# nhcha6/embodied-object-detection

Hardware: AMD Instinct MI355X
Metric: frames/sec (640x640, implicit_memory); frames/sec/GPU = value / n_gpus (higher is better)
Workload: dtype f32

## Files before the change

embodied_object_detection_amd/build.py:

```python
from __future__ import annotations

import os
import subprocess
import sys

HERE = os.path.dirname(os.path.abspath(__file__))
CSRC = os.path.join(HERE, "csrc")
LIB = os.path.join(HERE, "libeod_hip.so")
SOURCES = ["conv_igemm.hip", "conv_fp32.hip", "conv_pointwise.hip", "conv_bf16x3.hip", "conv_f16.hip", "elementwise.hip", "roi_align.hip", "select.hip", "heads.hip", "memory.hip", "semmap.hip", "place.hip", "regions.hip", "inventory.hip", "memory_read.hip", "memory_backward.hip", "conv_wgrad.hip", "train_losses.hip", "describe.hip", "relations.hip"]
ARCH = "gfx950"


def _stale() -> bool:
    if not os.path.exists(LIB):
        return True
    t = os.path.getmtime(LIB)
    deps = [os.path.join(CSRC, f) for f in os.listdir(CSRC)] + [os.path.join(HERE, "..", "include", h) for h in ("eod_hip.h", "eod_place.h", "eod_regions.h", "eod_inventory.h", "eod_describe.h", "eod_relations.h")]
    return any(os.path.getmtime(d) > t for d in deps if os.path.exists(d))


def _usage_file(src: str) -> str:
    return os.path.join(HERE, "build", src.replace(".hip", ".usage.txt"))


def resource_usage() -> dict:
    import re
    out = {}
    for src in SOURCES:
        f = _usage_file(src)
        if not os.path.exists(f):
            continue
        cur = None
        for line in open(f):
            m = re.search(r"Function Name: (\S+)", line)
            if m:
                cur = out.setdefault(m.group(1), {})
                continue
            for key, pat in (("vgprs", r"\bVGPRs: (\d+)"), ("scratch", r"ScratchSize \[bytes/lane\]: (\d+)"),
                             ("occupancy", r"Occupancy \[waves/SIMD\]: (\d+)"), ("lds", r"LDS Size \[bytes/block\]: (\d+)")):
                m = re.search(pat, line)
                if m and cur is not None:
                    cur[key] = int(m.group(1))
    return out


def scratch_offenders(usage: dict = None) -> list:
    usage = resource_usage() if usage is None else usage
    return sorted(k for k, v in usage.items() if v.get("scratch", 0) > 0)


def build(force: bool = False, verbose: bool = True) -> str:
    if not force and not _stale():
        return LIB
    hipcc = os.environ.get("HIPCC", "/opt/rocm/bin/hipcc")
    objs = []
    procs = []
    os.makedirs(os.path.join(HERE, "build"), exist_ok=True)
    for src in SOURCES:
        obj = os.path.join(HERE, "build", src.replace(".hip", ".o"))
        cmd = [hipcc, f"--offload-arch={ARCH}", "-O3", "-fPIC", "-std=c++17", "-Wall", "-Wno-unused-function",
               "-ffp-contract=on", "-Rpass-analysis=kernel-resource-usage", "-c", os.path.join(CSRC, src), "-o", obj]
        if verbose:
            print(" ".join(cmd), flush=True)
        procs.append((src, subprocess.Popen(cmd, stderr=open(_usage_file(src), "w"))))
        objs.append(obj)
    failed = [s for s, p in procs if p.wait() != 0]
    for src in SOURCES:
        skip = 0
        held = []
        for line in open(_usage_file(src)):
            if line.startswith("In file included from"):
                held.append(line)
                continue
            trace, held = held, []
            if "kernel-resource-usage" in line:
                skip = 2 if "Function Name" in line else 0
                continue
            sys.stderr.writelines(trace)
            if skip and (line.lstrip()[:1].isdigit() or line.strip().startswith("|")):
                skip -= 1
                continue
            skip = 0
            if line.strip():
                sys.stderr.write(line)
    if failed:
        raise RuntimeError(f"hipcc failed for {failed}")
    bad = scratch_offenders()
    if bad:
        raise RuntimeError("kernels that use scratch memory (register spills / an argument struct copied to private memory): " + ", ".join(bad))
    cmd = [hipcc, f"--offload-arch={ARCH}", "-shared", "-fPIC", "-o", LIB] + objs
    if verbose:
        print(" ".join(cmd), flush=True)
    subprocess.check_call(cmd)
    return LIB


if __name__ == "__main__":
    build(force="--force" in sys.argv)
    print(LIB)
```

embodied_object_detection_amd/csrc/conv_common.h:

```cpp
#pragma once
#include "eod_common.h"
#include "conv_border_order.h"
#include "../../include/eod_hip.h"

namespace eodconv {


struct ConvArgs {
  const float* x;
  const float* w;
  const float* bias;
  const float* res;
  const float* gate;
  float* y;
  float* partial;
  const int* m_count;
  int m_unit;
  int m_segs, seg_rows;
  const float* fuse_w;
  const int* out_units;
  float fuse_b;
  int N, H, W, Cin, OH, OW, Cout, KH, KW, stride, pad, Kpad;
  int M, nchunks, splitk, cps;
  int relu, res_mode, in_relu, out_mode;
  int tiles_m, tiles_n;
  float out_scale;
  int nlv;
  int lv_off[EOD_MAX_LEVELS + 1], lv_h[EOD_MAX_LEVELS], lv_w[EOD_MAX_LEVELS];
  unsigned x_bytes, w_bytes;
  const void* w3;
  unsigned w3_bytes;
  const void* wh;
  unsigned wh_bytes;
  double* gn_partial;
  int gn_groups;
  float* y2;
  int split_n;
  FastDiv div_ow, div_oh, div_cd, div_row;
  int border;
  FastDiv div_bh, div_bw, div_bi;
};

__device__ __forceinline__ int conv_row_limit(const ConvArgs& p, int M) {
  if (p.m_count && p.m_segs <= 1) {
    const int lim = *p.m_count * p.m_unit;
    M = lim < M ? lim : M;
  }
  return M;
}

__device__ __forceinline__ bool conv_row_active(const ConvArgs& p, int m) {
  if (!p.m_count || p.m_segs <= 1) return true;
  const int s = m / p.seg_rows;
  return m - s * p.seg_rows < p.m_count[s] * p.m_unit;
}

__device__ __forceinline__ bool conv_tile_active(const ConvArgs& p, int m0, int bm) {
  if (!p.m_count || p.m_segs <= 1) return true;
  const int last = (m0 + bm - 1 < p.M ? m0 + bm - 1 : p.M - 1);
  const int s0 = m0 / p.seg_rows, s1 = last / p.seg_rows;
  if (m0 - s0 * p.seg_rows < p.m_count[s0] * p.m_unit) return true;
  for (int s = s0 + 1; s <= s1; ++s)
    if (p.m_count[s] > 0) return true;
  return false;
}

__device__ __forceinline__ int border_rois(const ConvArgs& p) {
  const int c = *p.m_count;
  return c < p.N ? c : p.N;
}
__device__ __forceinline__ int border_storage_row(const ConvArgs& p, int m, int rois) {
  const BorderRow b = border_row(m, rois, p.OH, p.OW, p.div_ow, p.div_bh, p.div_bw, p.div_bi);
  return (b.img * p.OH + b.oy) * p.OW + b.ox;
}

template <bool GATE = false>
__device__ __forceinline__ float epilogue_store(const ConvArgs& p, float v, int m, int n) {
  int co = n;
  size_t oidx;
  if (p.out_mode == 1) {
    const int Cd = p.Cout >> 2;
    const int quad = (int)fdiv((unsigned)n, p.div_cd);
    co = n - quad * Cd;
    const int dy = quad >> 1, dx = quad & 1;
    const int t = (int)fdiv((unsigned)m, p.div_ow);
    const int ox = m - t * p.OW;
    const int img = (int)fdiv((unsigned)t, p.div_oh);
    const int oy = t - img * p.OH;
    oidx = ((size_t)(img * 2 * p.OH + 2 * oy + dy) * (2 * p.OW) + (2 * ox + dx)) * Cd + co;
  } else {
    oidx = (size_t)m * p.Cout + n;
  }
  if (p.bias) v += p.bias[co];
  v *= p.out_scale;
  if (p.res_mode == 1) {
    v += p.res[(size_t)m * p.Cout + n];
  } else if (p.res_mode == 2) {
    const int t = (int)fdiv((unsigned)m, p.div_ow);
    const int ox = m - t * p.OW;
    const int img = (int)fdiv((unsigned)t, p.div_oh);
    const int oy = t - img * p.OH;
    const int rh = p.OH >> 1, rw = p.OW >> 1;
    v += p.res[((size_t)(img * rh + (oy >> 1)) * rw + (ox >> 1)) * p.Cout + n];
  }
  if (p.split_n > 0) {
    if (n >= p.split_n) {
      if (p.relu) v = fmaxf(v, 0.0f);
      p.y2[(size_t)m * (p.Cout - p.split_n) + (n - p.split_n)] = v;
    } else {
      p.y[(size_t)m * p.split_n + n] = v;
    }
    return v;
  }
  if (p.relu) v = fmaxf(v, 0.0f);
  if (GATE && p.gate && !(p.gate[oidx] > 0.0f)) v = 0.0f;
  p.y[oidx] = v;
  return v;
}

__device__ __forceinline__ unsigned long long tap_mask(int iy0, int ix0, int hh, int ww, int KH, int KW) {
  unsigned long long mask = 0;
  int tp = 0;
  for (int ky = 0; ky < KH; ++ky) {
    const bool rok = (unsigned)(iy0 + ky) < (unsigned)hh;
    for (int kx = 0; kx < KW; ++kx, ++tp) {
      const bool ok = rok && ((unsigned)(ix0 + kx) < (unsigned)ww);
      mask |= (unsigned long long)ok << tp;
    }
  }
  return mask;
}

template <int TM, int TN, bool GATE = false, bool BORDER = false>
__device__ __forceinline__ void store_wave_tiles(const ConvArgs& p, const f32x16 (&acc)[TM][TN], int m_base, int n_base, int M, int z,
                                                 int lane) {
  const int half = lane >> 5;
  const int rois = BORDER ? border_rois(p) : 0;
#pragma unroll
  for (int i = 0; i < TM; ++i) {
#pragma unroll
    for (int j = 0; j < TN; ++j) {
      const int n = n_base + j * 32 + (lane & 31);
#pragma unroll
      for (int r = 0; r < 16; ++r) {
        const int row = (r & 3) + 8 * (r >> 2) + 4 * half;
        const int m = m_base + i * 32 + row;
        if (m < M && n < p.Cout && conv_row_active(p, m)) {
          const float v = acc[i][j][r];
          if (BORDER) {
            epilogue_store<GATE>(p, v, border_storage_row(p, m, rois), n);
          } else if (p.splitk > 1) {
            p.partial[((size_t)z * p.M + m) * p.Cout + n] = v;
          } else {
            epilogue_store<GATE>(p, v, m, n);
          }
        }
      }
    }
  }
}

void launch_conv_fp32(const ConvArgs& a, int tile, int bk, bool tap4, dim3 grid, hipStream_t s, int lds_reserve = 0, int prefetch2 = 0);
void launch_conv_bf16x3(const ConvArgs& a, int tile, dim3 grid, hipStream_t s);
void launch_conv_wavek(const ConvArgs& a, int nw, dim3 grid, hipStream_t s);
void launch_conv_pointwise(const ConvArgs& a, int np, dim3 grid, hipStream_t s);
void launch_split_weights(const float* w, void* out, int Cout, int Kpad, hipStream_t s);
void launch_conv_f16(const ConvArgs& a, int tile, int bk, dim3 grid, hipStream_t s);
void launch_half_weights(const float* w, void* out, int Cout, int Kpad, hipStream_t s);

}
```

embodied_object_detection_amd/csrc/conv_igemm.hip:

```cpp
#include "conv_common.h"
#include "../../include/eod_hip.h"
#include <atomic>
#include <cstdlib>
#include <cstring>

namespace {

using namespace eodconv;

template <int VEC>
__global__ __launch_bounds__(256) void conv_splitk_reduce_kernel(ConvArgs p) {
  EOD_CHAIN_PRIO();
  const int M = conv_row_limit(p, p.M);
  const unsigned per_row = (unsigned)p.Cout / VEC;
  const unsigned total = (unsigned)M * per_row;
  const size_t slab = (size_t)p.M * p.Cout;
  for (unsigned idx = blockIdx.x * blockDim.x + threadIdx.x; idx < total; idx += gridDim.x * blockDim.x) {
    const unsigned m = fdiv(idx, p.div_row);
    if (!conv_row_active(p, (int)m)) continue;
    const unsigned n = (idx - m * per_row) * VEC;
    const float* src = p.partial + (size_t)m * p.Cout + n;
    if (VEC == 4) {
      f32x4 v = {0.f, 0.f, 0.f, 0.f};
      for (int zb = 0; zb < p.splitk; zb += 4) {
        f32x4 t[4];
#pragma unroll
        for (int j = 0; j < 4; ++j)
          if (zb + j < p.splitk) t[j] = *reinterpret_cast<const f32x4*>(src + (size_t)(zb + j) * slab);
#pragma unroll
        for (int j = 0; j < 4; ++j)
          if (zb + j < p.splitk) v += t[j];
      }
      epilogue_store<true>(p, v.x, (int)m, (int)n);
      epilogue_store<true>(p, v.y, (int)m, (int)n + 1);
      epilogue_store<true>(p, v.z, (int)m, (int)n + 2);
      epilogue_store<true>(p, v.w, (int)m, (int)n + 3);
    } else {
      float v = 0.f;
      for (int z = 0; z < p.splitk; ++z) v += src[z * slab];
      epilogue_store<true>(p, v, (int)m, (int)n);
    }
  }
}

#define EOD_GN_ROWS 32
__global__ __launch_bounds__(256) void conv_splitk_reduce_gn_kernel(ConvArgs p) {
  EOD_CHAIN_PRIO();
  __shared__ double red[4][64][2];
  int level = 0, first_chunk = 0;
  for (;;) {
    const int rows = p.lv_off[level + 1] - p.lv_off[level];
    const int nch = (rows + EOD_GN_ROWS - 1) / EOD_GN_ROWS;
    if ((int)blockIdx.x < first_chunk + nch || level + 1 >= p.nlv) break;
    first_chunk += nch;
    ++level;
  }
  const int r0 = p.lv_off[level] + ((int)blockIdx.x - first_chunk) * EOD_GN_ROWS;
  const int r1 = min(r0 + EOD_GN_ROWS, p.lv_off[level + 1]);
  const int C = p.Cout;
  const int c4 = C >> 2;
  const int nsub = 256 / c4;
  const int col = threadIdx.x % c4, sub = threadIdx.x / c4;
  const int cpg4 = (C / p.gn_groups) >> 2;
  const size_t slab = (size_t)p.M * C;
  double s = 0.0, q = 0.0;
  for (int r = r0 + sub; r < r1; r += nsub) {
    const float* src = p.partial + (size_t)r * C + col * 4;
    f32x4 v = {0.f, 0.f, 0.f, 0.f};
    for (int zb = 0; zb < p.splitk; zb += 4) {
      f32x4 t[4];
#pragma unroll
      for (int j = 0; j < 4; ++j)
        if (zb + j < p.splitk) t[j] = *reinterpret_cast<const f32x4*>(src + (size_t)(zb + j) * slab);
#pragma unroll
      for (int j = 0; j < 4; ++j)
        if (zb + j < p.splitk) v += t[j];
    }
    const double o0 = (double)epilogue_store<true>(p, v.x, r, col * 4 + 0);
    const double o1 = (double)epilogue_store<true>(p, v.y, r, col * 4 + 1);
    const double o2 = (double)epilogue_store<true>(p, v.z, r, col * 4 + 2);
    const double o3 = (double)epilogue_store<true>(p, v.w, r, col * 4 + 3);
    s += o0; q += o0 * o0;
    s += o1; q += o1 * o1;
    s += o2; q += o2 * o2;
    s += o3; q += o3 * o3;
  }
  for (int off = 1; off < cpg4; off <<= 1) {
    s += __shfl_xor(s, off, 64);
    q += __shfl_xor(q, off, 64);
  }
  if ((col % cpg4) == 0) {
    red[sub][col / cpg4][0] = s;
    red[sub][col / cpg4][1] = q;
  }
  __syncthreads();
  if ((int)threadIdx.x < p.gn_groups) {
    double ts = 0.0, tq = 0.0;
    for (int u = 0; u < nsub; ++u) {
      ts += red[u][threadIdx.x][0];
      tq += red[u][threadIdx.x][1];
    }
    p.gn_partial[((size_t)blockIdx.x * p.gn_groups + threadIdx.x) * 2 + 0] = ts;
    p.gn_partial[((size_t)blockIdx.x * p.gn_groups + threadIdx.x) * 2 + 1] = tq;
  }
}

std::atomic<int>& math_mode() {
  static std::atomic<int> v([] {
    const char* e = getenv("EOD_CONV_MATH");
    if (e && strcmp(e, "bf16x3") == 0) return EOD_MATH_BF16X3;
    if (e && strcmp(e, "f16") == 0) return EOD_MATH_F16;
    return EOD_MATH_FP32;
  }());
  return v;
}

struct Plan {
  int tile;
  int bk;
  int glds;
  int bm, bn, tiles_m, tiles_n, splitk, cps, nchunks;
  int wavek;
  int pw_np;
  int border;
};

constexpr int kForcePointwise = 30;

int effective_math(const EodConvDesc* d) { return d->math > 0 ? d->math - 1 : math_mode().load(std::memory_order_relaxed); }

bool pointwise_eligible(const EodConvDesc* d) {
  return effective_math(d) == EOD_MATH_FP32 && d->KH == 1 && d->KW == 1 && d->stride == 1 && d->pad == 0 && d->levels <= 0 && !d->tap4 &&
         d->Cin == d->Kpad && (d->Cin == 64 || d->Cin == 128 || d->Cin == 256) && d->Cout % 64 == 0 && d->out_mode == 0 &&
         (d->res_mode == 0 || d->res_mode == 1) && !d->in_relu && !d->gate && !d->m_count && d->split_n == 0 && !d->gn_partial &&
         d->lds_reserve == 0;
}

constexpr int kForceBorder = 43;
constexpr bool kBorderAuto = true;

bool border_eligible(const EodConvDesc* d) {
  return effective_math(d) == EOD_MATH_FP32 && d->KH == 3 && d->KW == 3 && d->stride == 1 && d->pad == 1 && d->levels <= 0 && !d->tap4 &&
         d->m_count && d->m_segments <= 1 && d->m_unit == d->OH * d->OW && d->OH >= 3 && d->OW >= 3 && d->Cin % 32 == 0 &&
         d->out_mode == 0 && d->res_mode == 0 && !d->in_relu && !d->gate && d->split_n == 0 && !d->gn_partial && d->prefetch2 == 0;
}

Plan make_plan(const EodConvDesc* d, int M) {
  static const int cfg[5][2] = {{128, 128}, {128, 64}, {64, 64}, {256, 128}, {64, 256}};
  Plan pl{};
  int pick = 2;
  const int ft = d->force_tile % 10, fbk = d->force_tile / 10;
  const bool half_ok = !d->tap4 && !d->in_relu;
  const bool f16_forced = (fbk == 8 || fbk == 9) && half_ok;
  if (f16_forced) pick = ft == 4 ? 3 : 2;
  else if (ft >= 1 && ft <= 3) pick = ft - 1;
  else if (ft == 4 && fbk == 5 && half_ok) pick = 3;
  const bool bk64_ok = !d->tap4 && d->Cin % 64 == 0 && d->Kpad % 64 == 0;
  pl.glds = f16_forced ? 3 : ((fbk == 5 && half_ok) ? 2 : 0);
  const int Mp = (d->plan_rows > 0 && d->plan_rows < M) ? d->plan_rows : M;
  const int math = effective_math(d);
  if (d->force_tile == 0 && math == EOD_MATH_F16 && half_ok) {
    pl.glds = 3;
    pick = (long)((Mp + 255) / 256) * ((d->Cout + 127) / 128) >= 256 ? 3 : 2;
  }
  if (d->force_tile == 0 && math == EOD_MATH_BF16X3 && half_ok) {
    pl.glds = 2;
    const long t128 = (long)((Mp + 127) / 128) * ((d->Cout + 127) / 128);
    const long t256 = (long)((Mp + 255) / 256) * ((d->Cout + 127) / 128);
    pick = t256 >= 256 ? 3 : (t128 >= 512 ? 0 : 2);
  }
  if (d->out_mode == 2) {
    pick = 4;
    pl.glds = 0;
  }
  if (d->gate) {
    const bool f16_gated = d->math == EOD_MATH_F16 + 1 && half_ok && d->levels <= 0 && (d->force_tile == 0 || f16_forced);
    pick = 2;
    pl.glds = f16_gated ? 3 : 0;
  }
  if (pl.glds == 3) pl.bk = (fbk == 8 && d->Cin % 64 == 0) ? 64 : 32;
  else pl.bk = (pl.glds == 0 && d->out_mode != 2 && fbk == 2 && bk64_ok) ? 64 : 32;
  const int nchunks = d->Kpad / pl.bk;
  pl.nchunks = nchunks;
  pl.tile = pick + 1;
  pl.bm = cfg[pick][0];
  pl.bn = cfg[pick][1];
  pl.tiles_m = (M + pl.bm - 1) / pl.bm;
  pl.tiles_n = (d->Cout + pl.bn - 1) / pl.bn;
  const long tiles = (long)((Mp + pl.bm - 1) / pl.bm) * pl.tiles_n;
  int splitk = 1;
  if (d->out_mode == 2) {
    splitk = 1;
  } else if (d->force_splitk > 0) {
    splitk = d->force_splitk;
  } else if (pl.glds == 0 && !d->tap4 && nchunks >= 8 &&
             ((d->force_tile == 6 || d->force_tile == 7) ||
              (tiles < 256 && nchunks <= 192 && pl.bk == 32 && d->force_tile == 0 &&
               ((Mp <= 512 && nchunks / (nchunks >= 64 ? 8 : 4) >= 8) || nchunks >= 128)))) {
    pl.wavek = d->force_tile == 6 ? 4 : (d->force_tile == 7 ? 8 : (nchunks >= 64 ? 8 : 4));
    pl.bk = 32;
    pl.nchunks = d->Kpad / 32;
    pl.bm = pl.bn = 32;
    pl.tiles_m = (M + 31) / 32;
    pl.tiles_n = (d->Cout + 31) / 32;
  } else if (tiles < 256 && nchunks >= 8) {
    const int target = (nchunks >= 128 && Mp <= 512) ? 1792 : 512;
    int want = (int)((target + tiles - 1) / tiles);
    int maxs = nchunks / 4;
    splitk = want < maxs ? want : maxs;
    if (splitk < 1) splitk = 1;
  } else if (tiles >= 256 && tiles <= 1024 && d->m_count == nullptr && nchunks >= 18) {
    double best = 1e30;
    for (int sct = 1; sct <= 4; ++sct) {
      if (nchunks / sct < 9) break;
      const double est = (double)((tiles * sct + 255) / 256) / sct + (sct > 1 ? 0.12 : 0.0);
      if (est < best - 1e-9) {
        best = est;
        splitk = sct;
      }
    }
  }
  if (splitk > nchunks) splitk = nchunks;
  pl.cps = (nchunks + splitk - 1) / splitk;
  pl.splitk = (nchunks + pl.cps - 1) / pl.cps;
  const bool pw_forced = d->force_tile == kForcePointwise && d->force_splitk <= 1;
  const bool pw_auto = d->force_tile == 0 && d->force_splitk == 0 && pointwise_eligible(d) && pl.splitk == 1 && !pl.wavek && tiles >= 256 &&
                       !(d->Kpad == 256 && d->Cout < 1024);
  if (pw_forced || pw_auto) {
    const int panels = d->Cout / 64;
    const long row_tiles = (Mp + 63) / 64;
    const long want = tiles >= 256 ? 512 : 1;
    int np = 1;
    for (int cand = 4; cand > 1; cand >>= 1)
      if (panels >= cand && row_tiles * ((panels + cand - 1) / cand) >= want) {
        np = cand;
        break;
      }
    pl.pw_np = np;
    pl.tile = 6;
    pl.glds = 0;
    pl.bk = 32;
    pl.nchunks = d->Kpad / 32;
    pl.bm = 64;
    pl.bn = 64 * np;
    pl.tiles_m = (M + 63) / 64;
    pl.tiles_n = (panels + np - 1) / np;
    pl.splitk = 1;
    pl.cps = pl.nchunks;
    pl.wavek = 0;
  }
  const bool border_forced = d->force_tile == kForceBorder && d->force_splitk <= 1;
  const bool border_auto = kBorderAuto && d->force_tile == 0 && border_eligible(d) && pl.glds == 0 && pl.tile == 3 && pl.bk == 32 &&
                           pl.splitk == 1 && !pl.wavek;
  if (border_forced) {
    pl.splitk = 1;
    pl.cps = pl.nchunks;
  }
  pl.border = (border_forced || border_auto) ? 1 : 0;
  return pl;
}

int total_rows(const EodConvDesc* d) { return d->levels > 0 ? d->level_off[d->levels] : d->N * d->OH * d->OW; }

int check_desc(const EodConvDesc* d) {
  if (!d || !d->x || !d->w || !d->y) return EOD_ERR_NULL;
  if (d->N <= 0 || d->Cin <= 0 || d->Cout <= 0) return EOD_ERR_BAD_DIMS;
  if (d->levels <= 0 && (d->H <= 0 || d->W <= 0 || d->OH <= 0 || d->OW <= 0)) return EOD_ERR_BAD_DIMS;
  if (d->KH <= 0 || d->KW <= 0 || d->stride <= 0 || d->pad < 0) return EOD_ERR_BAD_DIMS;
  if (d->Kpad % 32 != 0 || d->Kpad < d->KH * d->KW * d->Cin) return EOD_ERR_BAD_DIMS;
  if (d->tap4) {
    if (d->Cin != 4) return EOD_ERR_BAD_DIMS;
  } else {
    if (d->Cin % 32 != 0 || d->Kpad != d->KH * d->KW * d->Cin) return EOD_ERR_BAD_DIMS;
  }
  if (d->levels > 0) {
    if (d->levels > EOD_MAX_LEVELS || d->N != 1 || d->stride != 1 || d->KH != d->KW || d->pad != d->KH / 2 || d->tap4 || d->out_mode != 0 ||
        d->res_mode == 2 || d->level_off[0] != 0)
      return EOD_ERR_BAD_DIMS;
    for (int l = 0; l < d->levels; ++l)
      if (d->level_h[l] <= 0 || d->level_w[l] <= 0 || d->level_off[l + 1] - d->level_off[l] != d->level_h[l] * d->level_w[l])
        return EOD_ERR_BAD_DIMS;
  } else {
    if (d->OH != (d->H + 2 * d->pad - d->KH) / d->stride + 1) return EOD_ERR_BAD_DIMS;
    if (d->OW != (d->W + 2 * d->pad - d->KW) / d->stride + 1) return EOD_ERR_BAD_DIMS;
  }
  if (d->levels <= 0 && (long)d->N * d->H * d->W * d->Cin >= (1L << 29)) return EOD_ERR_BAD_DIMS;
  if ((long)d->Cout * d->Kpad >= (1L << 29)) return EOD_ERR_BAD_DIMS;
  if (d->KH * d->KW > 64) return EOD_ERR_BAD_DIMS;
  if ((long)total_rows(d) * (d->Cout > d->Cin ? d->Cout : d->Cin) >= (1L << 31)) return EOD_ERR_BAD_DIMS;
  if (d->out_mode == 1 && (d->Cout % 4 != 0)) return EOD_ERR_BAD_DIMS;
  if (d->out_mode == 2) {
    if (d->Cout != 1024 || d->KH != 1 || d->KW != 1 || d->stride != 1 || d->tap4 || d->levels > 0 || d->res_mode != 0 || d->in_relu ||
        d->force_splitk > 1)
      return EOD_ERR_BAD_DIMS;
    if (!d->fuse_w) return EOD_ERR_NULL;
  }
  if (d->out_mode < 0 || d->out_mode > 2) return EOD_ERR_BAD_DIMS;
  if (d->res_mode != 0 && !d->res) return EOD_ERR_NULL;
  if (d->res_mode == 2 && ((d->OH & 1) || (d->OW & 1))) return EOD_ERR_BAD_DIMS;
  if (d->m_count && d->m_unit <= 0) return EOD_ERR_BAD_DIMS;
  if (d->m_segments > 1) {
    if (!d->m_count || d->levels > 0 || d->out_mode == 2 || d->m_segments > EOD_MAX_BATCH || d->N % d->m_segments != 0)
      return EOD_ERR_BAD_DIMS;
    if (((long)(d->N / d->m_segments) * d->OH * d->OW) % d->m_unit != 0) return EOD_ERR_BAD_DIMS;
  }
  if (d->gate && (d->out_mode != 0 || d->split_n != 0 || d->gn_partial)) return EOD_ERR_BAD_DIMS;
  if (d->gate && d->force_tile != 0 && d->force_tile % 10 != 3 && d->force_tile != 6 && d->force_tile != 7) return EOD_ERR_BAD_DIMS;
  if (d->gate && d->force_tile / 10 == 5) return EOD_ERR_BAD_DIMS;
  if (d->gate && (d->force_tile / 10 == 8 || d->force_tile / 10 == 9) &&
      (d->math != EOD_MATH_F16 + 1 || d->force_tile % 10 != 3 || d->levels > 0 || d->tap4 || d->in_relu))
    return EOD_ERR_BAD_DIMS;
  if (d->math < 0 || d->math > EOD_MATH_F16 + 1) return EOD_ERR_BAD_DIMS;
  if ((d->force_tile / 10 == 8 || d->force_tile / 10 == 9) && d->force_tile % 10 != 3 && d->force_tile % 10 != 4) return EOD_ERR_BAD_DIMS;
  if (d->lds_reserve < 0 || d->lds_reserve > 48 * 1024) return EOD_ERR_BAD_DIMS;
  if (d->force_tile == kForcePointwise && (!pointwise_eligible(d) || d->force_splitk > 1)) return EOD_ERR_BAD_DIMS;
  if (d->force_tile == kForceBorder && (!border_eligible(d) || d->force_splitk > 1)) return EOD_ERR_BAD_DIMS;
  if (d->split_n != 0) {
    if (!d->y2) return EOD_ERR_NULL;
    if (d->split_n < 0 || d->split_n >= d->Cout || d->out_mode != 0 || d->res_mode != 0 || d->levels > 0 || d->gn_partial)
      return EOD_ERR_BAD_DIMS;
  }
  if (d->gn_partial) {
    const int cpg = d->gn_groups > 0 ? d->Cout / d->gn_groups : 0;
    if (d->levels <= 0 || d->m_count || d->out_mode != 0 || d->gn_groups <= 0 || d->gn_groups > 64 || d->Cout % d->gn_groups != 0 ||
        cpg > 64 || (cpg & (cpg - 1)) != 0 || cpg < 4 || d->Cout % 4 != 0 || d->Cout > 1024 || 256 % (d->Cout / 4) != 0 ||
        64 % (cpg / 4) != 0)
      return EOD_ERR_BAD_DIMS;
  }
  if (!eod_aligned16(d->x) || !eod_aligned16(d->w) || !eod_aligned16(d->w_split) || !eod_aligned16(d->w_half)) return EOD_ERR_ALIGN;
  return EOD_OK;
}

}

extern "C" int eod_set_conv_math(int mode) {
  if (mode != EOD_MATH_FP32 && mode != EOD_MATH_BF16X3 && mode != EOD_MATH_F16) return EOD_ERR_BAD_DIMS;
  return math_mode().exchange(mode);
}

extern "C" int eod_get_conv_math(void) { return math_mode().load(); }

extern "C" size_t eod_conv_split_weights_bytes(int Cout, int Kpad) {
  return (Cout > 0 && Kpad > 0 && Kpad % 32 == 0) ? (size_t)Cout * Kpad * 6 : 0;
}

extern "C" int eod_conv_split_weights_bf16x3(const float* w, int Cout, int Kpad, void* out, eod_stream_t stream) {
  if (!w || !out) return EOD_ERR_NULL;
  if (Cout <= 0 || Kpad <= 0 || Kpad % 32 != 0 || (long)Cout * Kpad * 6 >= (1L << 32)) return EOD_ERR_BAD_DIMS;
  if (!eod_aligned16(w) || !eod_aligned16(out)) return EOD_ERR_ALIGN;
  launch_split_weights(w, out, Cout, Kpad, static_cast<hipStream_t>(stream));
  return eod_launch_status();
}

extern "C" size_t eod_conv_half_weights_bytes(int Cout, int Kpad) {
  return (Cout > 0 && Kpad > 0 && Kpad % 32 == 0) ? (size_t)Cout * Kpad * 2 : 0;
}

extern "C" int eod_conv_half_weights(const float* w, int Cout, int Kpad, void* out, eod_stream_t stream) {
  if (!w || !out) return EOD_ERR_NULL;
  if (Cout <= 0 || Kpad <= 0 || Kpad % 32 != 0 || (long)Cout * Kpad >= (1L << 29)) return EOD_ERR_BAD_DIMS;
  if (!eod_aligned16(w) || !eod_aligned16(out)) return EOD_ERR_ALIGN;
  launch_half_weights(w, out, Cout, Kpad, static_cast<hipStream_t>(stream));
  return eod_launch_status();
}

extern "C" int eod_conv2d_gn_fused(const EodConvDesc* d) {
  EodConvDesc t = *d;
  t.gn_partial = nullptr;
  if (check_desc(&t) != EOD_OK) return 0;
  return make_plan(&t, total_rows(&t)).splitk > 1 ? 1 : 0;
}

extern "C" int eod_conv2d_plan(const EodConvDesc* d, EodConvPlan* out) {
  if (!out) return EOD_ERR_NULL;
  const int st = check_desc(d);
  if (st != EOD_OK) return st;
  const Plan pl = make_plan(d, total_rows(d));
  out->tile = pl.tile; out->bm = pl.bm; out->bn = pl.bn; out->bk = pl.bk;
  out->splitk = pl.splitk; out->cps = pl.cps; out->nchunks = pl.nchunks;
  out->wavek = pl.wavek; out->glds = pl.glds;
  out->tiles_m = pl.tiles_m; out->tiles_n = pl.tiles_n;
  out->gn_fused = (d->gn_partial && pl.splitk > 1) ? 1 : 0;
  return EOD_OK;
}

extern "C" size_t eod_conv2d_workspace_bytes(const EodConvDesc* d) {
  if (check_desc(d) != EOD_OK) return 0;
  const int M = total_rows(d);
  const Plan pl = make_plan(d, M);
  if (pl.splitk <= 1) return 0;
  return (size_t)pl.splitk * M * d->Cout * sizeof(float);
}

extern "C" int eod_conv2d(const EodConvDesc* d, eod_stream_t stream) {
  const int st = check_desc(d);
  if (st != EOD_OK) return st;
  hipStream_t s = static_cast<hipStream_t>(stream);
  ConvArgs a{};
  a.x = d->x; a.w = d->w; a.bias = d->bias; a.res = d->res; a.y = d->y;
  a.partial = d->workspace;
  a.m_count = d->m_count; a.m_unit = d->m_unit;
  a.m_segs = d->m_segments > 1 ? d->m_segments : 1;
  a.seg_rows = a.m_segs > 1 ? (d->N / d->m_segments) * d->OH * d->OW : 0;
  a.fuse_w = d->fuse_w; a.out_units = d->out_units; a.fuse_b = d->fuse_b;
  a.N = d->N; a.H = d->H; a.W = d->W; a.Cin = d->Cin; a.OH = d->OH; a.OW = d->OW; a.Cout = d->Cout;
  a.KH = d->KH; a.KW = d->KW; a.stride = d->stride; a.pad = d->pad; a.Kpad = d->Kpad;
  a.M = total_rows(d);
  a.div_ow = eod_make_fastdiv((unsigned)(d->OW > 0 ? d->OW : 1));
  a.div_oh = eod_make_fastdiv((unsigned)(d->OH > 0 ? d->OH : 1));
  a.div_row = eod_make_fastdiv((unsigned)(d->Cout % 4 == 0 ? d->Cout / 4 : d->Cout));
  a.div_cd = eod_make_fastdiv((unsigned)((d->Cout >> 2) > 0 ? (d->Cout >> 2) : 1));
  a.div_bh = eod_make_fastdiv((unsigned)(d->OH > 2 ? d->OH - 2 : 1));
  a.div_bw = eod_make_fastdiv((unsigned)(d->OW > 2 ? d->OW - 2 : 1));
  a.div_bi = eod_make_fastdiv((unsigned)(d->OH > 2 && d->OW > 2 ? (d->OH - 2) * (d->OW - 2) : 1));
  {
    const size_t xe = d->levels > 0 ? (size_t)d->level_off[d->levels] * d->Cin : (size_t)d->N * d->H * d->W * d->Cin;
    a.x_bytes = (unsigned)(xe * sizeof(float));
    a.w_bytes = (unsigned)((size_t)d->Cout * d->Kpad * sizeof(float));
    a.w3 = d->w_split;
    a.w3_bytes = (unsigned)((size_t)d->Cout * d->Kpad * 6);
    a.wh = d->w_half;
    a.wh_bytes = (unsigned)((size_t)d->Cout * d->Kpad * 2);
  }
  a.nlv = d->levels > 0 ? d->levels : 0;
  for (int l = 0; l < a.nlv; ++l) {
    a.lv_off[l] = d->level_off[l];
    a.lv_h[l] = d->level_h[l];
    a.lv_w[l] = d->level_w[l];
  }
  if (a.nlv) a.lv_off[a.nlv] = d->level_off[a.nlv];
  a.relu = d->relu; a.res_mode = d->res_mode; a.in_relu = d->in_relu; a.out_mode = d->out_mode;
  a.gate = d->gate;
  a.out_scale = d->out_scale;
  a.gn_partial = d->gn_partial;
  a.gn_groups = d->gn_groups;
  a.y2 = d->y2;
  a.split_n = d->split_n;
  const Plan pl = make_plan(d, a.M);
  if (d->gn_partial && pl.splitk <= 1) return EOD_ERR_BAD_DIMS;
  a.nchunks = pl.nchunks;
  a.splitk = pl.splitk; a.cps = pl.cps; a.tiles_m = pl.tiles_m; a.tiles_n = pl.tiles_n;
  a.border = pl.border;
  if (pl.splitk > 1) {
    const size_t need = (size_t)pl.splitk * a.M * a.Cout * sizeof(float);
    if (!d->workspace || d->workspace_bytes < need) return EOD_ERR_CAPACITY;
  }
  dim3 grid(pl.tiles_m * pl.tiles_n, pl.splitk);
  if (pl.border) grid.x = (pl.tiles_m + 7) / 8 * 8 * pl.tiles_n;
  if (pl.pw_np) launch_conv_pointwise(a, pl.pw_np, grid, s);
  else if (pl.wavek) launch_conv_wavek(a, pl.wavek, grid, s);
  else if (pl.glds == 3) launch_conv_f16(a, pl.tile, pl.bk, grid, s);
  else if (pl.glds == 2) launch_conv_bf16x3(a, pl.tile, grid, s);
  else launch_conv_fp32(a, pl.tile, pl.bk, d->tap4 != 0, grid, s, d->lds_reserve, d->prefetch2);
  if (pl.splitk > 1) {
    const size_t total = (size_t)a.M * a.Cout;
    const bool vec = a.Cout % 4 == 0;
    int blocks = (int)((total / (vec ? 4 : 1) + 255) / 256);
    if (blocks > 2048) blocks = 2048;
    if (blocks < 1) blocks = 1;
    if (a.gn_partial) {
      int chunks = 0;
      for (int l = 0; l < a.nlv; ++l) chunks += (a.lv_off[l + 1] - a.lv_off[l] + EOD_GN_ROWS - 1) / EOD_GN_ROWS;
      hipLaunchKernelGGL(conv_splitk_reduce_gn_kernel, dim3(chunks), dim3(256), 0, s, a);
    } else if (vec) hipLaunchKernelGGL(conv_splitk_reduce_kernel<4>, dim3(blocks), dim3(256), 0, s, a);
    else hipLaunchKernelGGL(conv_splitk_reduce_kernel<1>, dim3(blocks), dim3(256), 0, s, a);
  }
  return eod_launch_status();
}
```

Before: 325.9.

## Add narrow-Cout 3x3 conv kernel with in-block split-K reduction

Adds a dedicated kernel for 3x3 stride-1 FP32 convolutions with at most 8 output channels. It is chosen automatically whenever the planner would otherwise use split-K. Each block covers 64 rows, and its four waves each take a K partition. Weights are broadcast across lanes with readlane, and the partial sums are reduced in LDS inside the block. This removes the split-K workspace write and the separate reduction kernel that the generic tiled path uses for these heads, but it may lose parallelism when there are few rows.

```diff
diff --git a/embodied_object_detection_amd/build.py b/embodied_object_detection_amd/build.py
--- a/embodied_object_detection_amd/build.py
+++ b/embodied_object_detection_amd/build.py
@@ -7,7 +7,7 @@
 HERE = os.path.dirname(os.path.abspath(__file__))
 CSRC = os.path.join(HERE, "csrc")
 LIB = os.path.join(HERE, "libeod_hip.so")
-SOURCES = ["conv_igemm.hip", "conv_fp32.hip", "conv_pointwise.hip", "conv_bf16x3.hip", "conv_f16.hip", "elementwise.hip", "roi_align.hip", "select.hip", "heads.hip", "memory.hip", "semmap.hip", "place.hip", "regions.hip", "inventory.hip", "memory_read.hip", "memory_backward.hip", "conv_wgrad.hip", "train_losses.hip", "describe.hip", "relations.hip"]
+SOURCES = ["conv_igemm.hip", "conv_fp32.hip", "conv_pointwise.hip", "conv_narrow.hip", "conv_bf16x3.hip", "conv_f16.hip", "elementwise.hip", "roi_align.hip", "select.hip", "heads.hip", "memory.hip", "semmap.hip", "place.hip", "regions.hip", "inventory.hip", "memory_read.hip", "memory_backward.hip", "conv_wgrad.hip", "train_losses.hip", "describe.hip", "relations.hip"]
 ARCH = "gfx950"
 
 
diff --git a/embodied_object_detection_amd/csrc/conv_common.h b/embodied_object_detection_amd/csrc/conv_common.h
--- a/embodied_object_detection_amd/csrc/conv_common.h
+++ b/embodied_object_detection_amd/csrc/conv_common.h
@@ -164,6 +164,7 @@
 void launch_conv_bf16x3(const ConvArgs& a, int tile, dim3 grid, hipStream_t s);
 void launch_conv_wavek(const ConvArgs& a, int nw, dim3 grid, hipStream_t s);
 void launch_conv_pointwise(const ConvArgs& a, int np, dim3 grid, hipStream_t s);
+void launch_conv_narrow(const ConvArgs& a, dim3 grid, hipStream_t s);
 void launch_split_weights(const float* w, void* out, int Cout, int Kpad, hipStream_t s);
 void launch_conv_f16(const ConvArgs& a, int tile, int bk, dim3 grid, hipStream_t s);
 void launch_half_weights(const float* w, void* out, int Cout, int Kpad, hipStream_t s);
diff --git a/embodied_object_detection_amd/csrc/conv_igemm.hip b/embodied_object_detection_amd/csrc/conv_igemm.hip
--- a/embodied_object_detection_amd/csrc/conv_igemm.hip
+++ b/embodied_object_detection_amd/csrc/conv_igemm.hip
@@ -123,6 +123,7 @@
   int wavek;
   int pw_np;
   int border;
+  int narrow;
 };
 
 constexpr int kForcePointwise = 30;
@@ -143,6 +144,14 @@
   return effective_math(d) == EOD_MATH_FP32 && d->KH == 3 && d->KW == 3 && d->stride == 1 && d->pad == 1 && d->levels <= 0 && !d->tap4 &&
          d->m_count && d->m_segments <= 1 && d->m_unit == d->OH * d->OW && d->OH >= 3 && d->OW >= 3 && d->Cin % 32 == 0 &&
          d->out_mode == 0 && d->res_mode == 0 && !d->in_relu && !d->gate && d->split_n == 0 && !d->gn_partial && d->prefetch2 == 0;
+}
+
+constexpr int kForceNarrow = 44;
+
+bool narrow_eligible(const EodConvDesc* d) {
+  return effective_math(d) == EOD_MATH_FP32 && d->Cout <= 8 && d->KH == 3 && d->KW == 3 && d->stride == 1 && d->pad == 1 && !d->tap4 &&
+         d->Cin % 32 == 0 && !d->m_count && d->m_segments <= 1 && d->out_mode == 0 && d->res_mode == 0 && !d->in_relu && !d->gate &&
+         d->split_n == 0 && !d->gn_partial && d->lds_reserve == 0 && d->prefetch2 == 0;
 }
 
 Plan make_plan(const EodConvDesc* d, int M) {
@@ -257,6 +266,15 @@
     pl.cps = pl.nchunks;
   }
   pl.border = (border_forced || border_auto) ? 1 : 0;
+  const bool narrow_ok = narrow_eligible(d) && pl.glds == 0 && pl.tile == 3 && pl.bk == 32 && !pl.wavek && !pl.border;
+  if (narrow_ok && (d->force_tile == kForceNarrow || (d->force_tile == 0 && pl.splitk > 1))) {
+    pl.narrow = 1;
+    pl.tile = 7;
+    pl.bm = 64;
+    pl.bn = 8;
+    pl.tiles_m = (M + 63) / 64;
+    pl.tiles_n = 1;
+  }
   return pl;
 }
 
@@ -315,6 +333,7 @@
   if (d->lds_reserve < 0 || d->lds_reserve > 48 * 1024) return EOD_ERR_BAD_DIMS;
   if (d->force_tile == kForcePointwise && (!pointwise_eligible(d) || d->force_splitk > 1)) return EOD_ERR_BAD_DIMS;
   if (d->force_tile == kForceBorder && (!border_eligible(d) || d->force_splitk > 1)) return EOD_ERR_BAD_DIMS;
+  if (d->force_tile == kForceNarrow && !narrow_eligible(d)) return EOD_ERR_BAD_DIMS;
   if (d->split_n != 0) {
     if (!d->y2) return EOD_ERR_NULL;
     if (d->split_n < 0 || d->split_n >= d->Cout || d->out_mode != 0 || d->res_mode != 0 || d->levels > 0 || d->gn_partial)
@@ -368,7 +387,8 @@
   EodConvDesc t = *d;
   t.gn_partial = nullptr;
   if (check_desc(&t) != EOD_OK) return 0;
-  return make_plan(&t, total_rows(&t)).splitk > 1 ? 1 : 0;
+  const Plan pl = make_plan(&t, total_rows(&t));
+  return (pl.splitk > 1 && !pl.narrow) ? 1 : 0;
 }
 
 extern "C" int eod_conv2d_plan(const EodConvDesc* d, EodConvPlan* out) {
@@ -380,7 +400,7 @@
   out->splitk = pl.splitk; out->cps = pl.cps; out->nchunks = pl.nchunks;
   out->wavek = pl.wavek; out->glds = pl.glds;
   out->tiles_m = pl.tiles_m; out->tiles_n = pl.tiles_n;
-  out->gn_fused = (d->gn_partial && pl.splitk > 1) ? 1 : 0;
+  out->gn_fused = (d->gn_partial && pl.splitk > 1 && !pl.narrow) ? 1 : 0;
   return EOD_OK;
 }
 
@@ -388,7 +408,7 @@
   if (check_desc(d) != EOD_OK) return 0;
   const int M = total_rows(d);
   const Plan pl = make_plan(d, M);
-  if (pl.splitk <= 1) return 0;
+  if (pl.splitk <= 1 || pl.narrow) return 0;
   return (size_t)pl.splitk * M * d->Cout * sizeof(float);
 }
 
@@ -441,6 +461,10 @@
   a.nchunks = pl.nchunks;
   a.splitk = pl.splitk; a.cps = pl.cps; a.tiles_m = pl.tiles_m; a.tiles_n = pl.tiles_n;
   a.border = pl.border;
+  if (pl.narrow) {
+    launch_conv_narrow(a, dim3(pl.tiles_m), s);
+    return eod_launch_status();
+  }
   if (pl.splitk > 1) {
     const size_t need = (size_t)pl.splitk * a.M * a.Cout * sizeof(float);
     if (!d->workspace || d->workspace_bytes < need) return EOD_ERR_CAPACITY;
diff --git a/embodied_object_detection_amd/csrc/conv_narrow.hip b/embodied_object_detection_amd/csrc/conv_narrow.hip
--- /dev/null
+++ b/embodied_object_detection_amd/csrc/conv_narrow.hip
@@ -0,0 +1,134 @@
+#include "conv_operands.h"
+
+namespace eodconv {
+namespace {
+
+constexpr int kRows = 64;
+constexpr int kLS = 36;
+
+__device__ __forceinline__ float lane_value(float v, int l) { return __int_as_float(__builtin_amdgcn_readlane(__float_as_int(v), l)); }
+
+template <int NC, bool MULTI>
+__global__ __launch_bounds__(256) void conv_narrow_kernel(ConvArgs p) {
+  EOD_CHAIN_PRIO();
+  constexpr int NW = (NC + 1) / 2;
+  __shared__ __attribute__((aligned(16))) float tile[4][kRows * kLS];
+  __shared__ float sp[4][kRows * NC];
+  const int lane = threadIdx.x & 63;
+  const int wave = __builtin_amdgcn_readfirstlane((int)(threadIdx.x >> 6));
+  float* As = tile[wave];
+  const int M = p.M;
+  const int m0 = blockIdx.x * kRows;
+
+  const int lr = lane >> 3, lq = lane & 7;
+  unsigned a_voff[8], a_pitch[MULTI ? 8 : 1];
+  unsigned long long a_mask[8];
+#pragma unroll
+  for (int i = 0; i < 8; ++i) conv_row_address<MULTI>(p, m0 + lr + 8 * i, M, lq, a_voff[i], a_mask[i], a_pitch[MULTI ? i : 0]);
+  unsigned w_voff[NW];
+#pragma unroll
+  for (int i = 0; i < NW; ++i) {
+    const int n = 2 * i + (lane >> 5);
+    w_voff[i] = n < NC ? (unsigned)((n * p.Kpad + (lane & 31)) * 4) : 0xFFFFFFFFu;
+  }
+  const __amdgpu_buffer_rsrc_t rsrc_x = conv_buffer(p.x, p.x_bytes);
+  const __amdgpu_buffer_rsrc_t rsrc_w = conv_buffer(p.w, p.w_bytes);
+
+  float total[2] = {0.f, 0.f};
+  for (int first = 0; first < p.splitk; first += 4) {
+    const int part = first + wave;
+    if (part < p.splitk) {
+      int c_end;
+      const int c_begin = conv_chunk_range(p, p.cps, part, c_end);
+      ChunkWalker<32, MULTI> walk(p, c_begin);
+      f32x4 ga0[8], ga1[8];
+      float gw0[NW], gw1[NW];
+      auto load_chunk = [&](f32x4 (&ga)[8], float (&gw)[NW]) {
+        const TapInfo ti = walk.next(p);
+#pragma unroll
+        for (int i = 0; i < 8; ++i) ga[i] = conv_load_a<MULTI>(rsrc_x, ti, a_voff[i], a_mask[i], a_pitch[MULTI ? i : 0]);
+#pragma unroll
+        for (int i = 0; i < NW; ++i) gw[i] = __uint_as_float(__builtin_amdgcn_raw_buffer_load_b32(rsrc_w, w_voff[i], (int)ti.k0b, 0));
+      };
+      float a[NC], b[NC];
+#pragma unroll
+      for (int n = 0; n < NC; ++n) a[n] = b[n] = 0.f;
+      auto stage_and_multiply = [&](f32x4 (&ga)[8], float (&gw)[NW], bool more) {
+#pragma unroll
+        for (int i = 0; i < 8; ++i) *reinterpret_cast<f32x4*>(As + (lr + 8 * i) * kLS + 4 * lq) = ga[i];
+        float wl[NW];
+#pragma unroll
+        for (int i = 0; i < NW; ++i) wl[i] = gw[i];
+        __builtin_amdgcn_fence(__ATOMIC_RELEASE, "wavefront");
+        __builtin_amdgcn_wave_barrier();
+        __builtin_amdgcn_fence(__ATOMIC_ACQUIRE, "wavefront");
+        f32x4 xr[8];
+#pragma unroll
+        for (int j = 0; j < 8; ++j) xr[j] = *reinterpret_cast<const f32x4*>(As + lane * kLS + 4 * j);
+        __builtin_amdgcn_fence(__ATOMIC_RELEASE, "wavefront");
+        __builtin_amdgcn_wave_barrier();
+        __builtin_amdgcn_fence(__ATOMIC_ACQUIRE, "wavefront");
+        if (more) load_chunk(ga, gw);
+#pragma unroll
+        for (int g = 0; g < 4; ++g) {
+          const f32x4 lo = xr[2 * g], hi = xr[2 * g + 1];
+#pragma unroll
+          for (int n = 0; n < NC; ++n) {
+            const float wv = wl[n >> 1];
+            const int l0 = (n & 1) * 32 + 8 * g;
+            a[n] = fmaf(lo.x, lane_value(wv, l0 + 0), a[n]);
+            b[n] = fmaf(lo.y, lane_value(wv, l0 + 1), b[n]);
+            a[n] = fmaf(hi.x, lane_value(wv, l0 + 4), a[n]);
+            b[n] = fmaf(hi.y, lane_value(wv, l0 + 5), b[n]);
+            a[n] = fmaf(lo.z, lane_value(wv, l0 + 2), a[n]);
+            b[n] = fmaf(lo.w, lane_value(wv, l0 + 3), b[n]);
+            a[n] = fmaf(hi.z, lane_value(wv, l0 + 6), a[n]);
+            b[n] = fmaf(hi.w, lane_value(wv, l0 + 7), b[n]);
+          }
+        }
+      };
+      if (c_begin < c_end) load_chunk(ga0, gw0);
+      if (c_begin + 1 < c_end) load_chunk(ga1, gw1);
+      for (int chunk = c_begin; chunk < c_end; chunk += 2) {
+        stage_and_multiply(ga0, gw0, chunk + 2 < c_end);
+        if (chunk + 1 < c_end) stage_and_multiply(ga1, gw1, chunk + 3 < c_end);
+      }
+#pragma unroll
+      for (int n = 0; n < NC; ++n) sp[wave][lane * NC + n] = a[n] + b[n];
+    }
+    __syncthreads();
+    const int nparts = p.splitk - first < 4 ? p.splitk - first : 4;
+#pragma unroll
+    for (int u = 0; u < 2; ++u) {
+      const int idx = threadIdx.x + 256 * u;
+      if (idx < kRows * NC) {
+        if (p.splitk == 1) total[u] = sp[0][idx];
+        else
+          for (int z = 0; z < nparts; ++z) total[u] += sp[z][idx];
+      }
+    }
+    __syncthreads();
+  }
+#pragma unroll
+  for (int u = 0; u < 2; ++u) {
+    const int idx = threadIdx.x + 256 * u;
+    const int row = idx / NC, n = idx - row * NC;
+    if (idx < kRows * NC && m0 + row < M) epilogue_store<false>(p, total[u], m0 + row, n);
+  }
+}
+
+}
+
+void launch_conv_narrow(const ConvArgs& a, dim3 grid, hipStream_t s) {
+#define EOD_NARROW(NC)                                                                                        \
+  case NC:                                                                                                    \
+    if (a.nlv > 0) hipLaunchKernelGGL((conv_narrow_kernel<NC, true>), grid, dim3(256), 0, s, a);             \
+    else hipLaunchKernelGGL((conv_narrow_kernel<NC, false>), grid, dim3(256), 0, s, a);                      \
+    break;
+  switch (a.Cout) {
+    EOD_NARROW(1) EOD_NARROW(2) EOD_NARROW(3) EOD_NARROW(4) EOD_NARROW(5) EOD_NARROW(6) EOD_NARROW(7) EOD_NARROW(8)
+  }
+#undef EOD_NARROW
+}
+
+}
```

After: 324.0. About the same (-0.6%).
